# sgl-project/rbg

Measured on AMD Instinct MI355X. Metric: output tok/s (llama-3-8b P/D-disagg serving, KV migration over xGMI), higher is better.
Workload: dtype bf16; 1 GPU; model=llama-3-8b, global_batch=128, seq_len=2048, parallelism=pd1 (1 prefill + 1 decode, prefill colocated with decode0)

## Files before the change

rbg_amd/models/llama.py:

```python
from __future__ import annotations

import math
from dataclasses import dataclass
from typing import Optional

import torch
import torch.nn as nn

from .. import ops
from ..engine.config import ModelConfig
from ..engine.kv_cache import PagedKVCache


@dataclass
class ForwardBatch:
    mode: str
    positions: torch.Tensor
    slot_mapping: torch.Tensor
    cu_seqlens: Optional[torch.Tensor] = None
    cu_seqlens_k: Optional[torch.Tensor] = None
    kv_gather_slots: Optional[torch.Tensor] = None
    block_tables: Optional[torch.Tensor] = None
    context_lens: Optional[torch.Tensor] = None
    decode_num_splits: int = 0
# ... 67 lines not shown

    def recv_prev(self, shape, dtype, device) -> torch.Tensor:
        from ..parallel.comm import from_wire, wire_dtype
        t = torch.empty(shape, dtype=wire_dtype(dtype, device),
                        device=device)
        torch.distributed.recv(t, src=self._lane_rank(self.stage - 1))
        return from_wire(t, dtype)

    def broadcast_tokens(self, t: torch.Tensor) -> torch.Tensor:
        src = self.ranks[(self.size - 1) * self.tp_size]
        torch.distributed.broadcast(t, src=src, group=self.group)
        return t


class LlamaAttention(nn.Module):
    def __init__(self, cfg: ModelConfig, layer_idx: int, tp: TPContext,
                 device, dtype, gen):
        super().__init__()
        self.cfg = cfg
        self.layer_idx = layer_idx
        self.tp = tp
        assert cfg.num_heads % tp.size == 0 and cfg.num_kv_heads % tp.size == 0, \
            "TP degree must divide head counts"
        self.heads = cfg.num_heads // tp.size
        self.kv_heads = cfg.num_kv_heads // tp.size
        self.head_dim = cfg.head_dim
        self.scale = 1.0 / math.sqrt(cfg.head_dim)
        q_out = self.heads * cfg.head_dim
        kv_out = self.kv_heads * cfg.head_dim
        full_q = cfg.num_heads * cfg.head_dim
        full_kv = cfg.num_kv_heads * cfg.head_dim
        wq = _linear_weight(full_q, cfg.hidden_size, device, dtype, gen,
                            shard_dim=0, tp_size=tp.size, tp_rank=tp.rank)
        wk = _linear_weight(full_kv, cfg.hidden_size, device, dtype, gen,
                            shard_dim=0, tp_size=tp.size, tp_rank=tp.rank)
        wv = _linear_weight(full_kv, cfg.hidden_size, device, dtype, gen,
                            shard_dim=0, tp_size=tp.size, tp_rank=tp.rank)
        self.wqkv = nn.Parameter(torch.cat([wq, wk, wv], dim=0),
                                 requires_grad=False)
        self.wo = _linear_weight(cfg.hidden_size, full_q, device, dtype, gen,
                                 shard_dim=1, tp_size=tp.size,
                                 tp_rank=tp.rank)
        self.q_out, self.kv_out = q_out, kv_out
        self.q_norm = self.k_norm = None
        if cfg.qk_norm:
            self.q_norm = nn.Parameter(torch.ones(cfg.head_dim, device=device,
                                                  dtype=dtype),
                                       requires_grad=False)
            self.k_norm = nn.Parameter(torch.ones(cfg.head_dim, device=device,
                                                  dtype=dtype),
                                       requires_grad=False)

    def forward(self, x: torch.Tensor, batch: ForwardBatch,
                kv: PagedKVCache, cos_sin: torch.Tensor) -> torch.Tensor:
        T = x.shape[0]
        qkv = ops.linear(x, self.wqkv)
        q = qkv[:, :self.q_out]
        k = qkv[:, self.q_out:self.q_out + self.kv_out]
        v = qkv[:, self.q_out + self.kv_out:]
        if self.q_norm is not None:
            q = ops.rmsnorm(q.contiguous().view(-1, self.head_dim),
                            self.q_norm,
                            self.cfg.rms_eps).view(T, self.q_out)
            k = ops.rmsnorm(k.contiguous().view(-1, self.head_dim),
                            self.k_norm,
                            self.cfg.rms_eps).view(T, self.kv_out)
            v = v.clone(memory_format=torch.contiguous_format)
        key_cache = kv.key_cache(self.layer_idx)
        value_cache = kv.value_cache(self.layer_idx)
        fp8 = kv.fp8
        if fp8:
            ops.rope_store_kv(q, k, v, key_cache, value_cache, cos_sin,
                              batch.positions, batch.slot_mapping,
                              kv.k_scale_log2, kv.v_scale_log2)
        else:
            ops.rope_store_kv(q, k, v, key_cache, value_cache, cos_sin,
                              batch.positions, batch.slot_mapping)
        q3 = q.view(T, self.heads, self.head_dim)
        if batch.mode == "prefill":
            if fp8:
                if batch.kv_gather_slots is None:
                    raise RuntimeError("an fp8 KV pool prefills through the "
                                       "gather path: kv_gather_slots unset")
                k_full = ops.kv_gather_dequant(
                    key_cache, batch.kv_gather_slots, kv.k_scale_log2)
                v_full = ops.kv_gather_dequant(
                    value_cache, batch.kv_gather_slots, kv.v_scale_log2)
                o = ops.prefill_attention(q3, k_full, v_full,
                                          batch.cu_seqlens, self.scale,
                                          batch.cu_seqlens_k)
            elif batch.kv_gather_slots is not None:
                ps = key_cache.shape[2]
                slots = batch.kv_gather_slots.long()
                pages, offs = slots // ps, slots % ps
                k_full = key_cache[pages, :, offs]
                v_full = value_cache[pages, :, offs]
                o = ops.prefill_attention(q3, k_full, v_full,
                                          batch.cu_seqlens, self.scale,
                                          batch.cu_seqlens_k)
            else:
                o = ops.prefill_attention(
                    q3, k.view(T, self.kv_heads, self.head_dim),
                    v.view(T, self.kv_heads, self.head_dim),
                    batch.cu_seqlens, self.scale)
        elif fp8:
            o = ops.decode_attention(q3, key_cache, value_cache,
                                     batch.block_tables, batch.context_lens,
                                     self.scale,
                                     num_splits=batch.decode_num_splits,
                                     k_scale_log2=kv.k_scale_log2,
                                     v_scale_log2=kv.v_scale_log2)
        else:
            o = ops.decode_attention(q3, key_cache, value_cache,
                                     batch.block_tables, batch.context_lens,
                                     self.scale,
                                     num_splits=batch.decode_num_splits)
        out = ops.linear(o.view(T, self.q_out).contiguous(), self.wo)
        return self.tp.all_reduce(out)


class LlamaMLP(nn.Module):
    def __init__(self, cfg: ModelConfig, tp: TPContext, device, dtype, gen):
        super().__init__()
        self.tp = tp
        assert cfg.intermediate_size % tp.size == 0
        inter = cfg.intermediate_size // tp.size
        wg = _linear_weight(cfg.intermediate_size, cfg.hidden_size, device,
                            dtype, gen, shard_dim=0, tp_size=tp.size,
                            tp_rank=tp.rank)
        wu = _linear_weight(cfg.intermediate_size, cfg.hidden_size, device,
                            dtype, gen, shard_dim=0, tp_size=tp.size,
                            tp_rank=tp.rank)
        self.w_gate_up = nn.Parameter(torch.cat([wg, wu], dim=0),
                                      requires_grad=False)
        self.w_down = _linear_weight(cfg.hidden_size, cfg.intermediate_size,
                                     device, dtype, gen, shard_dim=1,
                                     tp_size=tp.size, tp_rank=tp.rank)
        self.inter = inter

    def forward(self, x: torch.Tensor) -> torch.Tensor:
        gu = ops.linear(x, self.w_gate_up)
        h = ops.silu_mul(gu)
        return self.tp.all_reduce(ops.linear(h, self.w_down))


class LlamaLayer(nn.Module):
    def __init__(self, cfg: ModelConfig, layer_idx: int, tp: TPContext,
                 device, dtype, gen):
        super().__init__()
        self.attn = LlamaAttention(cfg, layer_idx, tp, device, dtype, gen)
        self.mlp = LlamaMLP(cfg, tp, device, dtype, gen)
        self.input_norm = nn.Parameter(
            torch.ones(cfg.hidden_size, device=device, dtype=dtype),
            requires_grad=False)
        self.post_norm = nn.Parameter(
            torch.ones(cfg.hidden_size, device=device, dtype=dtype),
            requires_grad=False)
        self.eps = cfg.rms_eps

    def forward(self, x: torch.Tensor, residual: Optional[torch.Tensor],
                batch: ForwardBatch, kv: PagedKVCache,
                cos_sin: torch.Tensor):
        if residual is None:
            residual = x.clone()
            h = ops.rmsnorm(x, self.input_norm, self.eps)
        else:
            ops.fused_add_rmsnorm(x, residual, self.input_norm, self.eps)
            h = x
        h = self.attn(h, batch, kv, cos_sin)
        ops.fused_add_rmsnorm(h, residual, self.post_norm, self.eps)
        h = self.mlp(h)
        return h, residual


class LlamaForCausalLM(nn.Module):
    def __init__(self, cfg: ModelConfig, device: torch.device,
                 tp: Optional[TPContext] = None, base_seed: int = 1234,
                 pp: Optional[PPContext] = None):
        super().__init__()
        self.cfg = cfg
        self.tp = tp or TPContext()
        self.pp = pp or PPContext()
        self.base_seed = base_seed
        self.device = device
        dtype = torch.bfloat16
        self.dtype = dtype

        def _gen(tag: int) -> torch.Generator:
            g = torch.Generator(device=device)
            g.manual_seed(base_seed * 1000003 + tag)
            return g

        L = cfg.num_layers
        assert L % self.pp.size == 0, "PP degree must divide layer count"
        per = L // self.pp.size
        self.layer_start = self.pp.stage * per
        self.layer_end = self.layer_start + per
        self.embed = None
        if self.pp.first:
            self.embed = nn.Parameter(
                torch.empty(cfg.vocab_size, cfg.hidden_size, device=device,
                            dtype=dtype).normal_(0, 0.02, generator=_gen(0)),
                requires_grad=False)
        self.layers = nn.ModuleList([
            LlamaLayer(cfg, i - self.layer_start, self.tp, device, dtype,
                       _gen(1 + i))
            for i in range(self.layer_start, self.layer_end)])
        self.final_norm = None
        self.lm_head = None
        if self.pp.last:
            self.final_norm = nn.Parameter(
                torch.ones(cfg.hidden_size, device=device, dtype=dtype),
                requires_grad=False)
            self.lm_head = _linear_weight(cfg.vocab_size, cfg.hidden_size,
                                          device, dtype, _gen(L + 1))
        self.cos_sin = ops.build_cos_sin_table(
            cfg.head_dim, cfg.max_position, cfg.rope_theta,
            device=device)

    @property
    def num_local_layers(self) -> int:
        return self.layer_end - self.layer_start

    @torch.inference_mode()
    def forward(self, tokens: torch.Tensor, batch: ForwardBatch,
                kv: PagedKVCache,
                hidden: Optional[torch.Tensor] = None) -> torch.Tensor:
        if self.pp.first:
            x = self.embed[tokens.long()]
        else:
            assert hidden is not None, "non-first PP stage needs hidden"
            x = hidden
        residual = None
        for layer in self.layers:
            x, residual = layer(x, residual, batch, kv, self.cos_sin)
        x = x + residual
        if not self.pp.last:
            return x
        x = ops.rmsnorm(x, self.final_norm, self.cfg.rms_eps)
        return x

    @torch.inference_mode()
    def logits(self, hidden: torch.Tensor,
               gather_idx: Optional[torch.Tensor] = None) -> torch.Tensor:
        if gather_idx is not None:
            hidden = hidden[gather_idx.long()]
        return torch.nn.functional.linear(hidden, self.lm_head).float()

    def reload_weights(self, seed: int) -> None:
        fresh = LlamaForCausalLM(self.cfg, self.device, self.tp,
                                 base_seed=seed, pp=self.pp)
        with torch.no_grad():
            for p, q in zip(self.parameters(), fresh.parameters()):
                p.copy_(q)
        del fresh
        if self.device.type == "cuda":
            torch.cuda.empty_cache()
        if self.tp.size > 1:
            torch.distributed.barrier(group=self.tp.group)
```

rbg_amd/ops/__init__.py:

```python
from __future__ import annotations

import os

import torch

from . import reference

_hip = None
_hip_err: Exception | None = None
try:
    from . import _hip_ops as _hip
except Exception as e:
    _hip_err = e

HAVE_HIP = _hip is not None


def _check_stale() -> None:
    import hashlib
    here = os.path.dirname(os.path.abspath(__file__))
    stamp = os.path.join(here, "_hip_ops.srchash")
    if not os.path.exists(stamp):
        return
    h = hashlib.sha256()
    hip_dir = os.path.join(here, "hip")
    for name in sorted(os.listdir(hip_dir)):
        if name.endswith("_hip.hip"):
            continue
        if name.endswith((".hip", ".cpp", ".h")):
            with open(os.path.join(hip_dir, name), "rb") as f:
                h.update(name.encode() + b"\0" + f.read() + b"\0")
    with open(stamp) as f:
        recorded = f.read().strip()
    if recorded and recorded != h.hexdigest():
        raise RuntimeError(
            "rbg_amd HIP extension is STALE: kernel sources changed after "
            "the last build.  Rebuild in-tree: PYTORCH_ROCM_ARCH=gfx950 "
            "python setup.py build_ext --inplace")


if HAVE_HIP and torch.cuda.is_available():
    _check_stale()


def _require_hip():
    if _hip is None:
        raise RuntimeError(
            "rbg_amd HIP extension is not built but a GPU tensor was passed. "
            "Build it in-tree: PYTORCH_ROCM_ARCH=gfx950 python setup.py "
            f"build_ext --inplace (import error: {_hip_err!r})")
    return _hip


def _on_gpu(t: torch.Tensor) -> bool:
    return t.is_cuda


SKINNY_GEMM = int(os.environ.get("RBG_SKINNY_GEMM", "1"))


def linear(x: torch.Tensor, w: torch.Tensor) -> torch.Tensor:
    if (SKINNY_GEMM and _on_gpu(x) and x.dim() == 2 and
            x.dtype == torch.bfloat16 and 1 <= x.shape[0] <= 128 and
            w.shape[0] % 32 == 0 and x.shape[1] % 512 == 0 and
            (w.shape[0] <= 4608 or
             (x.shape[0] <= 64 and w.shape[0] <= 8192))):
        return _require_hip().skinny_gemm(
            x if x.is_contiguous() else x.contiguous(), w)
    return torch.nn.functional.linear(x, w)


def rmsnorm(x: torch.Tensor, weight: torch.Tensor, eps: float) -> torch.Tensor:
    if _on_gpu(x):
        return _require_hip().rmsnorm(x, weight, eps)
    return reference.rmsnorm(x, weight, eps)


def fused_add_rmsnorm(x: torch.Tensor, residual: torch.Tensor,
                      weight: torch.Tensor, eps: float) -> None:
    if _on_gpu(x):
        _require_hip().fused_add_rmsnorm(x, residual, weight, eps)
        return
    reference.fused_add_rmsnorm(x, residual, weight, eps)


def silu_mul(x: torch.Tensor) -> torch.Tensor:
    if _on_gpu(x):
        return _require_hip().silu_mul(x)
    return reference.silu_mul(x)


FP8 = torch.float8_e4m3fn
KV_CACHE_DTYPES = reference.KV_CACHE_DTYPES
KV_SCALE_LOG2_RANGE = reference.KV_SCALE_LOG2_RANGE
check_kv_scale_log2 = reference.check_kv_scale_log2


def _is_fp8_pair(key_cache, value_cache) -> bool:
    if key_cache.dtype != value_cache.dtype:
        raise ValueError("key_cache is %s but value_cache is %s" % (
            key_cache.dtype, value_cache.dtype))
    return key_cache.dtype == FP8


def rope_store_kv(q, k, v, key_cache, value_cache, cos_sin, positions,
                  slot_mapping, k_scale_log2: int = 0,
                  v_scale_log2: int = 0) -> None:
    if _is_fp8_pair(key_cache, value_cache):
        check_kv_scale_log2(k_scale_log2, "kv_k_scale_log2")
        check_kv_scale_log2(v_scale_log2, "kv_v_scale_log2")
        if _on_gpu(q):
            _require_hip().rope_store_kv_fp8(
                q, k, v, key_cache, value_cache, cos_sin, positions,
                slot_mapping, k_scale_log2, v_scale_log2)
            return
        reference.rope_store_kv(q, k, v, key_cache, value_cache, cos_sin,
                                positions, slot_mapping, k_scale_log2,
                                v_scale_log2)
        return
    if _on_gpu(q):
        _require_hip().rope_store_kv(q, k, v, key_cache, value_cache,
                                     cos_sin, positions, slot_mapping)
# ... 102 lines not shown
```

rbg_amd/ops/hip/bindings.cpp:

```cpp
#include <torch/extension.h>
#include <ATen/hip/HIPContext.h>

#include <hip/hip_runtime.h>

#include <algorithm>
#include <cmath>
#include <cstring>
#include <vector>

extern "C" {
void launch_rmsnorm(void*, void*, const void*, float, int, int, hipStream_t);
void launch_fused_add_rmsnorm(void*, void*, const void*, float, int, int,
                              hipStream_t);
void launch_silu_mul(void*, const void*, int, int, hipStream_t);
void launch_rope_store_kv(void*, void*, const void*, void*, void*,
                          const void*, const void*, const void*, int, int,
                          int, int, int, int, int, hipStream_t);
void launch_decode_attention(void*, void*, void*, const void*, const void*,
                             const void*, const void*, const void*, float,
                             int, int, int, int, int, int, int, int,
                             hipStream_t);
void launch_prefill_attention(void*, const void*, const void*, const void*,
                              const void*, const void*, float, int, int, int,
                              int, int, int, hipStream_t);
void launch_mfma_probe(void*, const void*, const void*, int, int, hipStream_t);
void launch_mfma_probe32(void*, const void*, const void*, int, int, int,
                         hipStream_t);
void launch_skinny_gemm(void*, void*, const void*, const void*, int, int,
                        int, int, hipStream_t);
void launch_reduce_splits(void*, const void*, int, long, hipStream_t);
void launch_kv_peer_copy(void*, const void*, const void*, const void*, int,
                         int, int, long, long, long, long, hipStream_t);
void launch_xgmi_allreduce(void*, const void*, void**, void**, int, int,
                           long, hipStream_t);
void launch_sample(void*, void*, const void*, const void*, const void*,
                   const void*, const void*, const void*, const void*, int,
                   int, hipStream_t);
void launch_rope_store_kv_fp8(void*, void*, const void*, void*, void*,
                              const void*, const void*, const void*, int, int,
                              int, int, int, int, float, float, hipStream_t);
void launch_kv_gather_dequant(void*, const void*, const void*, long, int, int,
                              int, float, hipStream_t);
void launch_decode_attention_fp8(void*, void*, void*, const void*, const void*,
                                 const void*, const void*, const void*, float,
                                 float, int, int, int, int, int, int,
                                 hipStream_t);
long xgmi_allreduce_signal_bytes();
long xgmi_allreduce_error_offset();
long xgmi_allreduce_counter_offset();
}

namespace {

hipStream_t current_stream() {
  return at::hip::getCurrentHIPStream().stream();
}

void check_bf16_contig(const torch::Tensor& t, const char* name) {
  TORCH_CHECK(t.is_cuda(), name, " must be on GPU");
  TORCH_CHECK(t.scalar_type() == torch::kBFloat16, name, " must be bf16");
  TORCH_CHECK(t.is_contiguous(), name, " must be contiguous");
}

void check_i32_gpu(const torch::Tensor& t, const char* name) {
  TORCH_CHECK(t.is_cuda(), name, " must be on GPU");
  TORCH_CHECK(t.scalar_type() == torch::kInt32, name, " must be int32");
  TORCH_CHECK(t.is_contiguous(), name, " must be contiguous");
}

void check_kv_caches(const torch::Tensor& key_cache,
                     const torch::Tensor& value_cache) {
  check_bf16_contig(key_cache, "key_cache");
  check_bf16_contig(value_cache, "value_cache");
  TORCH_CHECK(key_cache.dim() == 4,
              "key_cache must be [pages, KVH, page_size, head_dim]");
  TORCH_CHECK(value_cache.sizes() == key_cache.sizes(),
              "key_cache/value_cache shape mismatch");
  const int64_t page_size = key_cache.size(2);
  TORCH_CHECK(page_size > 0 && (page_size & (page_size - 1)) == 0,
              "page_size must be a power of two");
  TORCH_CHECK(key_cache.size(1) > 0, "cache needs at least one KV head");
  TORCH_CHECK(key_cache.size(3) > 0 && key_cache.size(3) % 8 == 0,
              "cache head_dim must be a multiple of 8");
// ... 317 lines not shown
  rowsliced3(q, "q");
  rowsliced3(k, "k");
  rowsliced3(v, "v");
  TORCH_CHECK(k.stride(0) == v.stride(0), "k/v stride mismatch");
  TORCH_CHECK(q.size(2) == 128, "head_dim must be 128");
  TORCH_CHECK(block_info.scalar_type() == torch::kInt32, "block_info int32");
  TORCH_CHECK(seq_lens.scalar_type() == torch::kInt32, "seq_lens int32");
  const int nblocks = block_info.size(0);
  const int num_q_heads = q.size(1);
  const int num_kv_heads = k.size(1);
  auto out = torch::empty({q.size(0), (int64_t)num_q_heads, (int64_t)128},
                          q.options());
  launch_prefill_attention(out.data_ptr(), q.data_ptr(), k.data_ptr(),
                           v.data_ptr(), block_info.data_ptr(),
                           seq_lens.data_ptr(), (float)scale, nblocks,
                           num_q_heads, num_kv_heads, (int)swz,
                           (int)q.stride(0), (int)k.stride(0),
                           current_stream());
  return out;
}

torch::Tensor mfma_probe(torch::Tensor a, torch::Tensor b, int64_t a_split,
                         int64_t b_split) {
  auto d = torch::zeros({16, 16}, a.options().dtype(torch::kFloat32));
  launch_mfma_probe(d.data_ptr(), a.data_ptr(), b.data_ptr(), (int)a_split,
                    (int)b_split, current_stream());
  return d;
}

torch::Tensor mfma_probe32(torch::Tensor a, torch::Tensor b, int64_t a_split,
                           int64_t b_split, int64_t dmap) {
  auto d = torch::zeros({32, 32}, a.options().dtype(torch::kFloat32));
  launch_mfma_probe32(d.data_ptr(), a.data_ptr(), b.data_ptr(), (int)a_split,
                      (int)b_split, (int)dmap, current_stream());
  return d;
}

}

static int pick_gemm_splits(int N, int K) {
  const int n_groups = N >> 5;
  for (int s : {8, 4, 2})
    if (n_groups * s <= 512 && n_groups * s >= 192 && K % (s * 256) == 0)
      return s;
  for (int s : {4, 2})
    if (n_groups * s >= 128 && K % (s * 256) == 0) return s;
  return 1;
}

bool skinny_gemm_supported(int64_t M, int64_t N, int64_t K) {
  return M >= 1 && M <= 256 && (N % 32) == 0 && (K % 256) == 0;
}

torch::Tensor skinny_gemm(torch::Tensor a, torch::Tensor w,
                          int64_t force_splits = 0) {
  check_bf16_contig(a, "a");
  check_bf16_contig(w, "w");
  TORCH_CHECK(a.dim() == 2 && w.dim() == 2, "a and w must be 2-D");
  TORCH_CHECK(a.device() == w.device(), "a/w device mismatch");
  const int64_t M = a.size(0), K = a.size(1), N = w.size(0);
  TORCH_CHECK(w.size(1) == K, "K mismatch");
  TORCH_CHECK(skinny_gemm_supported(M, N, K), "unsupported skinny shape");
  TORCH_CHECK(force_splits == 0 || force_splits == 1 || force_splits == 2 ||
                  force_splits == 4 || force_splits == 8,
              "force_splits must be 0 (auto), 1, 2, 4 or 8");
  TORCH_CHECK(force_splits == 0 || K % (force_splits * 256) == 0,
              "K must be a multiple of force_splits * 256");
  auto c = torch::empty({M, N}, a.options());
  const int splits = force_splits > 0 ? (int)force_splits
                                      : pick_gemm_splits((int)N, (int)K);
  torch::Tensor ws;
  void* wsp = nullptr;
  if (splits > 1) {
    ws = torch::empty({splits, M, N}, a.options().dtype(torch::kFloat32));
    wsp = ws.data_ptr();
  }
  launch_skinny_gemm(c.data_ptr(), wsp, a.data_ptr(), w.data_ptr(), (int)M,
                     (int)N, (int)K, splits, current_stream());
  if (splits > 1)
    launch_reduce_splits(c.data_ptr(), wsp, splits, (long)(M * N),
                         current_stream());
  return c;
}

std::vector<torch::Tensor> sample(torch::Tensor logits,
                                  torch::Tensor temperature,
                                  torch::Tensor top_k, torch::Tensor top_p,
                                  torch::Tensor min_p, torch::Tensor seed,
                                  torch::Tensor pos) {
  TORCH_CHECK(logits.is_cuda(), "logits must be on GPU");
  TORCH_CHECK(logits.scalar_type() == torch::kFloat32, "logits must be fp32");
  TORCH_CHECK(logits.dim() == 2, "logits must be [n, V]");
  TORCH_CHECK(logits.is_contiguous(), "logits must be contiguous");
  const int64_t n = logits.size(0), V = logits.size(1);
  TORCH_CHECK(V >= 1, "V must be >= 1");
  TORCH_CHECK(V <= INT32_MAX && n <= INT32_MAX, "n and V must fit int32");
  auto check_param = [&](const torch::Tensor& t, torch::ScalarType dt,
                         const char* name) {
    TORCH_CHECK(t.is_cuda() && t.device() == logits.device(), name,
                " must be on the logits' device");
    TORCH_CHECK(t.scalar_type() == dt, name, " has the wrong dtype");
    TORCH_CHECK(t.dim() == 1 && t.size(0) == n, name,
                " must have one entry per row");
    TORCH_CHECK(t.is_contiguous(), name, " must be contiguous");
  };
  check_param(temperature, torch::kFloat32, "temperature");
  check_param(top_k, torch::kInt32, "top_k");
  check_param(top_p, torch::kFloat32, "top_p");
  check_param(min_p, torch::kFloat32, "min_p");
  check_param(seed, torch::kInt64, "seed");
  check_param(pos, torch::kInt32, "pos");
  auto tokens = torch::empty({n}, logits.options().dtype(torch::kInt64));
  auto kept = torch::empty({n}, logits.options().dtype(torch::kInt32));
  if (n == 0) return {tokens, kept};
  launch_sample(tokens.data_ptr(), kept.data_ptr(), logits.data_ptr(),
                temperature.data_ptr(), top_k.data_ptr(), top_p.data_ptr(),
                min_p.data_ptr(), seed.data_ptr(), pos.data_ptr(), (int)n,
                (int)V, current_stream());
  return {tokens, kept};
}


torch::Tensor ipc_alloc_bf16(std::vector<int64_t> sizes) {
  int64_t numel = 1;
  for (auto s : sizes) numel *= s;
  void* ptr = nullptr;
  hipError_t err = hipMalloc(&ptr, numel * 2);
  TORCH_CHECK(err == hipSuccess, "hipMalloc(", numel * 2,
              " B) failed: ", hipGetErrorString(err));
  int dev = 0;
  (void)hipGetDevice(&dev);
  auto opts = torch::TensorOptions()
                  .dtype(torch::kBFloat16)
                  .device(torch::kCUDA, dev);
  return torch::from_blob(
      ptr, sizes, [](void* p) { (void)hipFree(p); }, opts);
// ... 99 lines not shown
  unsigned err_word = 0;
  char* base = reinterpret_cast<char*>(sig_ptr);
  (void)hipMemcpy(&err_word, base + xgmi_allreduce_error_offset(),
                  sizeof(unsigned), hipMemcpyDeviceToHost);
  return err_word;
}

torch::Tensor ar_dump_signals(int64_t sig_ptr) {
  long n = xgmi_allreduce_signal_bytes() / 4;
  auto t = torch::empty({n}, torch::TensorOptions().dtype(torch::kInt32));
  (void)hipMemcpy(t.data_ptr(), reinterpret_cast<void*>(sig_ptr), n * 4,
                  hipMemcpyDeviceToHost);
  return t;
}

torch::Tensor xgmi_allreduce(torch::Tensor inp,
                             std::vector<int64_t> sig_ptrs,
                             std::vector<int64_t> data_ptrs, int64_t rank) {
  check_bf16_contig(inp, "inp");
  const int world = (int)sig_ptrs.size();
  TORCH_CHECK(world >= 1 && world <= 8 &&
                  data_ptrs.size() == (size_t)world && rank >= 0 &&
                  rank < world,
              "bad world/rank");
  TORCH_CHECK(inp.numel() % 8 == 0, "numel must be a multiple of 8");
  auto out = torch::empty_like(inp);
  void* sp[8];
  void* dp[8];
  for (int i = 0; i < world; ++i) {
    sp[i] = reinterpret_cast<void*>(sig_ptrs[i]);
    dp[i] = reinterpret_cast<void*>(data_ptrs[i]);
  }
  launch_xgmi_allreduce(out.data_ptr(), inp.data_ptr(), sp, dp, world,
                        (int)rank, (long)inp.numel(), current_stream());
  return out;
}

PYBIND11_MODULE(TORCH_EXTENSION_NAME, m) {
  m.def("rmsnorm", &rmsnorm, "RMSNorm (bf16)");
  m.def("fused_add_rmsnorm", &fused_add_rmsnorm, "x,residual += ; rmsnorm");
  m.def("silu_mul", &silu_mul, "silu(gate)*up");
  m.def("rope_store_kv", &rope_store_kv, "RoPE + paged KV write");
  m.def("decode_attention", &decode_attention, "paged flash-decode");
  m.def("rope_store_kv_fp8", &rope_store_kv_fp8,
        "RoPE + quantising (e4m3) paged KV write");
  m.def("kv_gather_dequant", &kv_gather_dequant,
        "gather e4m3 cache rows by slot -> bf16 [Tkv, KVH, D]");
  m.def("decode_attention_fp8", &decode_attention_fp8,
        "paged flash-decode over an e4m3 cache (page-pair MFMA)");
  m.def("prefill_attention", &prefill_attention, "varlen causal flash prefill");
  m.def("mfma_probe", &mfma_probe, "MFMA layout probe");
  m.def("mfma_probe32", &mfma_probe32, "32x32x16 MFMA layout probe");
  m.def("skinny_gemm", &skinny_gemm, "decode-shape GEMM (M<=128)",
        py::arg("a"), py::arg("w"), py::arg("force_splits") = 0);
  m.def("sample", &sample,
        "seeded top-k/min-p/top-p Gumbel-max sampler -> (tokens, num_kept)");
  m.def("ipc_alloc_bf16", &ipc_alloc_bf16,
        "hipMalloc-backed bf16 tensor (IPC-exportable base allocation)",
        py::call_guard<py::gil_scoped_release>());
  m.def("ipc_alloc", &ipc_alloc,
        "hipMalloc-backed tensor of any dtype (IPC-exportable allocation)",
        py::call_guard<py::gil_scoped_release>());
  m.def("kv_ipc_export", &kv_ipc_export, "hipIpcGetMemHandle of a KV pool");
  m.def("kv_ipc_open", &kv_ipc_open,
        "map a peer KV pool (lazy xGMI peer access)",
        py::call_guard<py::gil_scoped_release>());
  m.def("kv_ipc_close", &kv_ipc_close, "unmap a peer KV pool",
        py::call_guard<py::gil_scoped_release>());
  m.def("kv_peer_copy", &kv_peer_copy,
        "gather local pages -> scatter into peer pool over xGMI",
        py::call_guard<py::gil_scoped_release>());
  m.def("ar_alloc_signals", &ar_alloc_signals,
        "uncached signal buffer for the xGMI all-reduce");
  m.def("ar_export_ptr", &ar_export_ptr, "hipIpc handle of a raw pointer");
  m.def("ar_error_flag", &ar_error_flag, "read the all-reduce error word");
  m.def("ar_dump_signals", &ar_dump_signals, "debug: dump the signal block");
  m.def("ar_counter_offset", &xgmi_allreduce_counter_offset);
  m.def("xgmi_allreduce", &xgmi_allreduce,
        "one-shot all-reduce over peer-mapped HBM (graph-capturable)");
}
```

rbg_amd/ops/hip/rmsnorm.hip:

```cpp
#include "common.h"

namespace {

template <bool FUSED_ADD>
__global__ void rmsnorm_kernel(__hip_bfloat16* __restrict__ out,
                               __hip_bfloat16* __restrict__ input,
                               __hip_bfloat16* __restrict__ residual,
                               const __hip_bfloat16* __restrict__ w,
                               const float eps, const int hidden) {
  const int row = blockIdx.x;
  const int tid = threadIdx.x;
  const int nthreads = blockDim.x;
  __shared__ float red[8];
  __shared__ float s_inv;

  __hip_bfloat16* in_row = input + (size_t)row * hidden;
  __hip_bfloat16* res_row =
      FUSED_ADD ? residual + (size_t)row * hidden : nullptr;
  __hip_bfloat16* out_row = out + (size_t)row * hidden;

  const int nvec = hidden / 8;
  float ss = 0.f;
  for (int i = tid; i < nvec; i += nthreads) {
    Bf16x8U xv;
    xv.u = *reinterpret_cast<const uint4*>(in_row + i * 8);
    if (FUSED_ADD) {
      Bf16x8U rv;
      rv.u = *reinterpret_cast<const uint4*>(res_row + i * 8);
#pragma unroll
      for (int j = 0; j < 8; ++j) {
        float s = bf2f(xv.e[j]) + bf2f(rv.e[j]);
        xv.e[j] = f2bf(s);
        ss += s * s;
      }
      *reinterpret_cast<uint4*>(res_row + i * 8) = xv.u;
    } else {
#pragma unroll
      for (int j = 0; j < 8; ++j) {
        float s = bf2f(xv.e[j]);
        ss += s * s;
      }
    }
  }
  const int lane = tid & 63, wave = tid >> 6;
  ss = wave_sum(ss);
  if (lane == 0) red[wave] = ss;
  __syncthreads();
  if (tid == 0) {
    float total = 0.f;
    for (int wv = 0; wv < (nthreads >> 6); ++wv) total += red[wv];
    s_inv = rsqrtf(total / hidden + eps);
  }
  __syncthreads();
  const float inv = s_inv;

  const __hip_bfloat16* src = FUSED_ADD ? res_row : in_row;
  for (int i = tid; i < nvec; i += nthreads) {
    Bf16x8U xv, wv, ov;
    xv.u = *reinterpret_cast<const uint4*>(src + i * 8);
    wv.u = *reinterpret_cast<const uint4*>(w + i * 8);
#pragma unroll
    for (int j = 0; j < 8; ++j)
      ov.e[j] = f2bf(bf2f(xv.e[j]) * inv * bf2f(wv.e[j]));
    *reinterpret_cast<uint4*>(out_row + i * 8) = ov.u;
  }
}

}

extern "C" {

void launch_rmsnorm(void* out, void* input, const void* weight, float eps,
                    int tokens, int hidden, hipStream_t stream) {
  dim3 grid(tokens), block(256);
  hipLaunchKernelGGL(rmsnorm_kernel<false>, grid, block, 0, stream,
                     (__hip_bfloat16*)out, (__hip_bfloat16*)input,
                     (__hip_bfloat16*)nullptr, (const __hip_bfloat16*)weight,
                     eps, hidden);
}

void launch_fused_add_rmsnorm(void* input, void* residual, const void* weight,
                              float eps, int tokens, int hidden,
                              hipStream_t stream) {
  dim3 grid(tokens), block(256);
  hipLaunchKernelGGL(rmsnorm_kernel<true>, grid, block, 0, stream,
                     (__hip_bfloat16*)input, (__hip_bfloat16*)input,
                     (__hip_bfloat16*)residual, (const __hip_bfloat16*)weight,
                     eps, hidden);
}

}
```

rbg_amd/ops/hip/skinny_gemm.hip:

```cpp
#include "common.h"

typedef __attribute__((ext_vector_type(8))) __bf16 gg_bf8;

DEV_INLINE gg_bf8 lds_frag(const __hip_bfloat16* p) {
  union { uint4 u; gg_bf8 v; } cvt;
  cvt.u = *reinterpret_cast<const uint4*>(p);
  return cvt.v;
}

#define SG_KSTEP 64
#define SG_LDS_PITCH (SG_KSTEP + 8)
#define SG_NT 256

template <int M_TILES, int SPLITS>
__global__ __launch_bounds__(SG_NT, 3) void skinny_gemm_kernel(
    const __hip_bfloat16* __restrict__ a,
    const __hip_bfloat16* __restrict__ w,
    __hip_bfloat16* __restrict__ c,
    float* __restrict__ ws,
    const int M, const int N, const int K) {
  const int n_groups = N >> 5;
  const int n_group = blockIdx.x % n_groups;
  const int split = blockIdx.x / n_groups;
  const int tid = threadIdx.x;
// ... 96 lines not shown
  __hip_bfloat16* buf1 = lds.stage[1];

  SG_ISSUE(0, wreg0, a00, a01, a02, a03, a04, a05, a06, a07);
  SG_ISSUE(1, wreg1, a10, a11, a12, a13, a14, a15, a16, a17);
  SG_WRITE(buf0, wreg0, a00, a01, a02, a03, a04, a05, a06, a07);
  SG_ISSUE(2, wreg0, a00, a01, a02, a03, a04, a05, a06, a07);

  for (int step = 0; step < nsteps; step += 2) {
    __syncthreads();
    compute(buf0);
    SG_WRITE(buf1, wreg1, a10, a11, a12, a13, a14, a15, a16, a17);
    SG_ISSUE(step + 3, wreg1, a10, a11, a12, a13, a14, a15, a16, a17);
    __syncthreads();
    compute(buf1);
    SG_WRITE(buf0, wreg0, a00, a01, a02, a03, a04, a05, a06, a07);
    SG_ISSUE(step + 4, wreg0, a00, a01, a02, a03, a04, a05, a06, a07);
  }
#undef SG_ISSUE
#undef SG_WRITE
#undef SG_ABASE
#undef SG_LD
#undef SG_AST

  __syncthreads();
#pragma unroll
  for (int mt = 0; mt < M_TILES; ++mt) {
    F32x4U u;
    u.v = acc[mt];
#pragma unroll
    for (int r = 0; r < 4; ++r)
      lds.red[wave][mt * 256 + r * 64 + lane] = u.e[r];
  }
  __syncthreads();

  const int elems = M_TILES * 256 * 2;
  for (int e = tid; e < elems; e += SG_NT) {
    const int nt = e >= M_TILES * 256;
    const int ee = e - nt * M_TILES * 256;
    const float v = lds.red[nt][ee] + lds.red[2 + nt][ee];
    const int l64 = ee & 63;
    const int reg = (ee >> 6) & 3;
    const int mt = ee >> 8;
    const int m = mt * 16 + ((l64 >> 4) << 2) + reg;
    if (m < M) {
      const int n = (n_group << 5) + (nt << 4) + (l64 & 15);
      if (SPLITS == 1)
        c[(size_t)m * N + n] = f2bf(v);
      else
        ws[((size_t)split * M + m) * N + n] = v;
    }
  }
}

__global__ void reduce_splits_kernel(const float* __restrict__ ws,
                                     __hip_bfloat16* __restrict__ c,
                                     const int splits, const long mn) {
  const long i = (long)blockIdx.x * blockDim.x + threadIdx.x;
  if (i >= mn) return;
  float v = 0.f;
  for (int s = 0; s < splits; ++s) v += ws[(size_t)s * mn + i];
  c[i] = f2bf(v);
}


extern "C" void launch_skinny_gemm(void* c, void* ws, const void* a,
                                   const void* w, int M, int N, int K,
                                   int splits, hipStream_t stream) {
  const dim3 grid((N >> 5) * splits), block(SG_NT);
  const __hip_bfloat16* ap = (const __hip_bfloat16*)a;
  const __hip_bfloat16* wp = (const __hip_bfloat16*)w;
  __hip_bfloat16* cp = (__hip_bfloat16*)c;
  float* wsp = (float*)ws;
  const int m_tiles = (M + 15) >> 4;

#define LAUNCH_MT(MT)                                                        \
  do {                                                                       \
    if (splits == 1)                                                         \
      skinny_gemm_kernel<MT, 1><<<grid, block, 0, stream>>>(                 \
          ap, wp, cp, nullptr, M, N, K);                                     \
    else if (splits == 2)                                                    \
      skinny_gemm_kernel<MT, 2><<<grid, block, 0, stream>>>(                 \
          ap, wp, cp, wsp, M, N, K);                                         \
    else if (splits == 4)                                                    \
      skinny_gemm_kernel<MT, 4><<<grid, block, 0, stream>>>(                 \
          ap, wp, cp, wsp, M, N, K);                                         \
    else                                                                     \
      skinny_gemm_kernel<MT, 8><<<grid, block, 0, stream>>>(                 \
          ap, wp, cp, wsp, M, N, K);                                         \
  } while (0)

  if (m_tiles <= 1) LAUNCH_MT(1);
  else if (m_tiles <= 2) LAUNCH_MT(2);
  else if (m_tiles <= 4) LAUNCH_MT(4);
  else if (m_tiles <= 8) LAUNCH_MT(8);
  else LAUNCH_MT(16);
#undef LAUNCH_MT
}

extern "C" void launch_reduce_splits(void* c, const void* ws, int splits,
                                     long mn, hipStream_t stream) {
  const int threads = 256;
  reduce_splits_kernel<<<dim3((mn + threads - 1) / threads), dim3(threads),
                         0, stream>>>((const float*)ws, (__hip_bfloat16*)c,
                                      splits, mn);
}
```

Baseline: 10380 tok/s.

## Fuse split-K reduction into add-RMSNorm and add wide-panel skinny GEMM

Folds the split-K partial-sum reduction into the following fused add+RMSNorm kernel, and moves each layer's next input norm into the MLP down-projection epilogue, so one reduce kernel and one norm launch per linear are removed. It also adds a 64-column, 512-thread skinny GEMM variant with double-buffered LDS staging, chosen automatically for M>32. The goal is fewer decode kernel launches and less memory traffic, at the cost of a new untested kernel path and more complex layer wiring when TP size is 1.

```diff
diff --git a/rbg_amd/models/llama.py b/rbg_amd/models/llama.py
--- a/rbg_amd/models/llama.py
+++ b/rbg_amd/models/llama.py
@@ -143,7 +143,8 @@
                                        requires_grad=False)
 
     def forward(self, x: torch.Tensor, batch: ForwardBatch,
-                kv: PagedKVCache, cos_sin: torch.Tensor) -> torch.Tensor:
+                kv: PagedKVCache, cos_sin: torch.Tensor,
+                add_norm=None) -> torch.Tensor:
         T = x.shape[0]
         qkv = ops.linear(x, self.wqkv)
         q = qkv[:, :self.q_out]
@@ -206,8 +207,10 @@
                                      batch.block_tables, batch.context_lens,
                                      self.scale,
                                      num_splits=batch.decode_num_splits)
-        out = ops.linear(o.view(T, self.q_out).contiguous(), self.wo)
-        return self.tp.all_reduce(out)
+        o = o.view(T, self.q_out).contiguous()
+        if add_norm is not None:
+            return ops.linear_add_rmsnorm(o, self.wo, *add_norm)
+        return self.tp.all_reduce(ops.linear(o, self.wo))
 
 
 class LlamaMLP(nn.Module):
@@ -229,9 +232,11 @@
                                      tp_size=tp.size, tp_rank=tp.rank)
         self.inter = inter
 
-    def forward(self, x: torch.Tensor) -> torch.Tensor:
+    def forward(self, x: torch.Tensor, add_norm=None) -> torch.Tensor:
         gu = ops.linear(x, self.w_gate_up)
         h = ops.silu_mul(gu)
+        if add_norm is not None:
+            return ops.linear_add_rmsnorm(h, self.w_down, *add_norm)
         return self.tp.all_reduce(ops.linear(h, self.w_down))
 
 
@@ -248,6 +253,9 @@
             torch.ones(cfg.hidden_size, device=device, dtype=dtype),
             requires_grad=False)
         self.eps = cfg.rms_eps
+        self.fuse_norms = False
+        self.next_input_norm: tuple = ()
+        self.input_prenormed = False
 
     def forward(self, x: torch.Tensor, residual: Optional[torch.Tensor],
                 batch: ForwardBatch, kv: PagedKVCache,
@@ -255,13 +263,21 @@
         if residual is None:
             residual = x.clone()
             h = ops.rmsnorm(x, self.input_norm, self.eps)
+        elif self.input_prenormed:
+            h = x
         else:
             ops.fused_add_rmsnorm(x, residual, self.input_norm, self.eps)
             h = x
-        h = self.attn(h, batch, kv, cos_sin)
-        ops.fused_add_rmsnorm(h, residual, self.post_norm, self.eps)
-        h = self.mlp(h)
-        return h, residual
+        if not self.fuse_norms:
+            h = self.attn(h, batch, kv, cos_sin)
+            ops.fused_add_rmsnorm(h, residual, self.post_norm, self.eps)
+            return self.mlp(h), residual
+        h = self.attn(h, batch, kv, cos_sin,
+                      add_norm=(residual, self.post_norm, self.eps))
+        if self.next_input_norm:
+            return self.mlp(h, add_norm=(residual, self.next_input_norm[0],
+                                         self.eps)), residual
+        return self.mlp(h), residual
 
 
 class LlamaForCausalLM(nn.Module):
@@ -297,6 +313,7 @@
             LlamaLayer(cfg, i - self.layer_start, self.tp, device, dtype,
                        _gen(1 + i))
             for i in range(self.layer_start, self.layer_end)])
+        self.link_norm_fusion(self.tp.size == 1)
         self.final_norm = None
         self.lm_head = None
         if self.pp.last:
@@ -308,6 +325,14 @@
         self.cos_sin = ops.build_cos_sin_table(
             cfg.head_dim, cfg.max_position, cfg.rope_theta,
             device=device)
+
+    def link_norm_fusion(self, on: bool) -> None:
+        layers = list(self.layers)
+        for i, layer in enumerate(layers):
+            nxt = layers[i + 1] if on and i + 1 < len(layers) else None
+            layer.fuse_norms = on
+            layer.input_prenormed = on and i > 0
+            layer.next_input_norm = () if nxt is None else (nxt.input_norm,)
 
     @property
     def num_local_layers(self) -> int:
diff --git a/rbg_amd/ops/__init__.py b/rbg_amd/ops/__init__.py
--- a/rbg_amd/ops/__init__.py
+++ b/rbg_amd/ops/__init__.py
@@ -60,14 +60,30 @@
 
 
 def linear(x: torch.Tensor, w: torch.Tensor) -> torch.Tensor:
-    if (SKINNY_GEMM and _on_gpu(x) and x.dim() == 2 and
-            x.dtype == torch.bfloat16 and 1 <= x.shape[0] <= 128 and
-            w.shape[0] % 32 == 0 and x.shape[1] % 512 == 0 and
-            (w.shape[0] <= 4608 or
-             (x.shape[0] <= 64 and w.shape[0] <= 8192))):
+    if _use_skinny_gemm(x, w):
         return _require_hip().skinny_gemm(
             x if x.is_contiguous() else x.contiguous(), w)
     return torch.nn.functional.linear(x, w)
+
+
+def _use_skinny_gemm(x: torch.Tensor, w: torch.Tensor) -> bool:
+    return bool(SKINNY_GEMM and _on_gpu(x) and x.dim() == 2 and
+                x.dtype == torch.bfloat16 and 1 <= x.shape[0] <= 128 and
+                w.shape[0] % 32 == 0 and x.shape[1] % 512 == 0 and
+                (w.shape[0] <= 4608 or
+                 (x.shape[0] <= 64 and w.shape[0] <= 8192)))
+
+
+def linear_add_rmsnorm(x: torch.Tensor, w: torch.Tensor,
+                       residual: torch.Tensor, norm_weight: torch.Tensor,
+                       eps: float) -> torch.Tensor:
+    if _use_skinny_gemm(x, w):
+        return _require_hip().skinny_gemm_add_rmsnorm(
+            x if x.is_contiguous() else x.contiguous(), w, residual,
+            norm_weight, eps)
+    h = linear(x, w)
+    fused_add_rmsnorm(h, residual, norm_weight, eps)
+    return h
 
 
 def rmsnorm(x: torch.Tensor, weight: torch.Tensor, eps: float) -> torch.Tensor:
diff --git a/rbg_amd/ops/hip/bindings.cpp b/rbg_amd/ops/hip/bindings.cpp
--- a/rbg_amd/ops/hip/bindings.cpp
+++ b/rbg_amd/ops/hip/bindings.cpp
@@ -28,7 +28,11 @@
                          hipStream_t);
 void launch_skinny_gemm(void*, void*, const void*, const void*, int, int,
                         int, int, hipStream_t);
+void launch_skinny_gemm_wide(void*, void*, const void*, const void*, int, int,
+                             int, int, hipStream_t);
 void launch_reduce_splits(void*, const void*, int, long, hipStream_t);
+void launch_fold_add_rmsnorm(void*, const void*, void*, const void*, float,
+                             int, int, int, hipStream_t);
 void launch_kv_peer_copy(void*, const void*, const void*, const void*, int,
                          int, int, long, long, long, long, hipStream_t);
 void launch_xgmi_allreduce(void*, const void*, void**, void**, int, int,
@@ -452,8 +456,19 @@
   return M >= 1 && M <= 256 && (N % 32) == 0 && (K % 256) == 0;
 }
 
-torch::Tensor skinny_gemm(torch::Tensor a, torch::Tensor w,
-                          int64_t force_splits = 0) {
+bool skinny_gemm_wide_supported(int64_t M, int64_t N) {
+  return M >= 1 && M <= 128 && (N % 64) == 0;
+}
+
+static int pick_gemm_panel(int64_t M, int64_t N) {
+  return M > 32 && skinny_gemm_wide_supported(M, N) ? 64 : 32;
+}
+
+namespace {
+
+int skinny_gemm_launch(const torch::Tensor& a, const torch::Tensor& w,
+                       int64_t force_splits, int64_t panel, torch::Tensor& c,
+                       torch::Tensor& ws) {
   check_bf16_contig(a, "a");
   check_bf16_contig(w, "w");
   TORCH_CHECK(a.dim() == 2 && w.dim() == 2, "a and w must be 2-D");
@@ -466,22 +481,74 @@
               "force_splits must be 0 (auto), 1, 2, 4 or 8");
   TORCH_CHECK(force_splits == 0 || K % (force_splits * 256) == 0,
               "K must be a multiple of force_splits * 256");
-  auto c = torch::empty({M, N}, a.options());
+  TORCH_CHECK(panel == 0 || panel == 32 || panel == 64,
+              "panel must be 0 (auto), 32 or 64");
+  TORCH_CHECK(panel != 64 || skinny_gemm_wide_supported(M, N),
+              "panel 64 needs M <= 128 and N % 64 == 0");
   const int splits = force_splits > 0 ? (int)force_splits
                                       : pick_gemm_splits((int)N, (int)K);
-  torch::Tensor ws;
+  if (panel == 0) panel = pick_gemm_panel(M, N);
+  void* cp = nullptr;
   void* wsp = nullptr;
   if (splits > 1) {
     ws = torch::empty({splits, M, N}, a.options().dtype(torch::kFloat32));
     wsp = ws.data_ptr();
+  } else {
+    c = torch::empty({M, N}, a.options());
+    cp = c.data_ptr();
   }
-  launch_skinny_gemm(c.data_ptr(), wsp, a.data_ptr(), w.data_ptr(), (int)M,
-                     (int)N, (int)K, splits, current_stream());
-  if (splits > 1)
-    launch_reduce_splits(c.data_ptr(), wsp, splits, (long)(M * N),
-                         current_stream());
+  (panel == 64 ? launch_skinny_gemm_wide : launch_skinny_gemm)(
+      cp, wsp, a.data_ptr(), w.data_ptr(), (int)M, (int)N, (int)K, splits,
+      current_stream());
+  return splits;
+}
+
+}
+
+torch::Tensor skinny_gemm(torch::Tensor a, torch::Tensor w,
+                          int64_t force_splits = 0, int64_t panel = 0) {
+  torch::Tensor c, ws;
+  const int splits = skinny_gemm_launch(a, w, force_splits, panel, c, ws);
+  if (splits > 1) {
+    c = torch::empty({a.size(0), w.size(0)}, a.options());
+    launch_reduce_splits(c.data_ptr(), ws.data_ptr(), splits,
+                         (long)c.numel(), current_stream());
+  }
   return c;
 }
+
+torch::Tensor skinny_gemm_add_rmsnorm(torch::Tensor a, torch::Tensor w,
+                                      torch::Tensor residual,
+                                      torch::Tensor norm_weight, double eps,
+                                      int64_t force_splits = 0,
+                                      int64_t panel = 0) {
+  check_bf16_contig(residual, "residual");
+  check_bf16_contig(norm_weight, "norm_weight");
+  TORCH_CHECK(a.dim() == 2 && w.dim() == 2, "a and w must be 2-D");
+  TORCH_CHECK(residual.dim() == 2 && residual.size(0) == a.size(0) &&
+                  residual.size(1) == w.size(0),
+              "residual must be [M, N]");
+  TORCH_CHECK(norm_weight.numel() == w.size(0),
+              "norm_weight must have N elements");
+  TORCH_CHECK(residual.device() == a.device() &&
+                  norm_weight.device() == a.device(),
+              "a/residual/norm_weight device mismatch");
+  torch::Tensor c, ws;
+  const int splits = skinny_gemm_launch(a, w, force_splits, panel, c, ws);
+  const int M = (int)a.size(0), N = (int)w.size(0);
+  if (splits == 1) {
+    launch_fused_add_rmsnorm(c.data_ptr(), residual.data_ptr(),
+                             norm_weight.data_ptr(), (float)eps, M, N,
+                             current_stream());
+    return c;
+  }
+  c = torch::empty({a.size(0), w.size(0)}, a.options());
+  launch_fold_add_rmsnorm(c.data_ptr(), ws.data_ptr(), residual.data_ptr(),
+                          norm_weight.data_ptr(), (float)eps, splits, M, N,
+                          current_stream());
+  return c;
+}
+
 
 std::vector<torch::Tensor> sample(torch::Tensor logits,
                                   torch::Tensor temperature,
@@ -687,7 +754,14 @@
   m.def("mfma_probe", &mfma_probe, "MFMA layout probe");
   m.def("mfma_probe32", &mfma_probe32, "32x32x16 MFMA layout probe");
   m.def("skinny_gemm", &skinny_gemm, "decode-shape GEMM (M<=128)",
-        py::arg("a"), py::arg("w"), py::arg("force_splits") = 0);
+        py::arg("a"), py::arg("w"), py::arg("force_splits") = 0,
+        py::arg("panel") = 0);
+  m.def("skinny_gemm_add_rmsnorm", &skinny_gemm_add_rmsnorm,
+        "skinny_gemm + fused_add_rmsnorm with the split-K fold inside the "
+        "norm kernel; returns h, updates residual in place",
+        py::arg("a"), py::arg("w"), py::arg("residual"),
+        py::arg("norm_weight"), py::arg("eps"), py::arg("force_splits") = 0,
+        py::arg("panel") = 0);
   m.def("sample", &sample,
         "seeded top-k/min-p/top-p Gumbel-max sampler -> (tokens, num_kept)");
   m.def("ipc_alloc_bf16", &ipc_alloc_bf16,
diff --git a/rbg_amd/ops/hip/rmsnorm.hip b/rbg_amd/ops/hip/rmsnorm.hip
--- a/rbg_amd/ops/hip/rmsnorm.hip
+++ b/rbg_amd/ops/hip/rmsnorm.hip
@@ -2,19 +2,24 @@
 
 namespace {
 
-template <bool FUSED_ADD>
+enum { NORM_PLAIN = 0, NORM_FUSED_ADD = 1, NORM_FOLD_ADD = 2 };
+
+template <int MODE, int SPLITS = 1>
 __global__ void rmsnorm_kernel(__hip_bfloat16* __restrict__ out,
                                __hip_bfloat16* __restrict__ input,
                                __hip_bfloat16* __restrict__ residual,
                                const __hip_bfloat16* __restrict__ w,
+                               const float* __restrict__ ws,
                                const float eps, const int hidden) {
+  constexpr bool FUSED_ADD = MODE != NORM_PLAIN;
   const int row = blockIdx.x;
   const int tid = threadIdx.x;
   const int nthreads = blockDim.x;
   __shared__ float red[8];
   __shared__ float s_inv;
 
-  __hip_bfloat16* in_row = input + (size_t)row * hidden;
+  __hip_bfloat16* in_row =
+      MODE == NORM_FOLD_ADD ? nullptr : input + (size_t)row * hidden;
   __hip_bfloat16* res_row =
       FUSED_ADD ? residual + (size_t)row * hidden : nullptr;
   __hip_bfloat16* out_row = out + (size_t)row * hidden;
@@ -23,7 +28,26 @@
   float ss = 0.f;
   for (int i = tid; i < nvec; i += nthreads) {
     Bf16x8U xv;
-    xv.u = *reinterpret_cast<const uint4*>(in_row + i * 8);
+    if (MODE == NORM_FOLD_ADD) {
+      const size_t mn = (size_t)gridDim.x * hidden;
+      const float* p = ws + (size_t)row * hidden + i * 8;
+      float4 lo[SPLITS], hi[SPLITS];
+#pragma unroll
+      for (int s = 0; s < SPLITS; ++s) {
+        lo[s] = *reinterpret_cast<const float4*>(p + s * mn);
+        hi[s] = *reinterpret_cast<const float4*>(p + s * mn + 4);
+      }
+      float v[8] = {0.f, 0.f, 0.f, 0.f, 0.f, 0.f, 0.f, 0.f};
+#pragma unroll
+      for (int s = 0; s < SPLITS; ++s) {
+        v[0] += lo[s].x; v[1] += lo[s].y; v[2] += lo[s].z; v[3] += lo[s].w;
+        v[4] += hi[s].x; v[5] += hi[s].y; v[6] += hi[s].z; v[7] += hi[s].w;
+      }
+#pragma unroll
+      for (int j = 0; j < 8; ++j) xv.e[j] = f2bf(v[j]);
+    } else {
+      xv.u = *reinterpret_cast<const uint4*>(in_row + i * 8);
+    }
     if (FUSED_ADD) {
       Bf16x8U rv;
       rv.u = *reinterpret_cast<const uint4*>(res_row + i * 8);
@@ -73,20 +97,36 @@
 void launch_rmsnorm(void* out, void* input, const void* weight, float eps,
                     int tokens, int hidden, hipStream_t stream) {
   dim3 grid(tokens), block(256);
-  hipLaunchKernelGGL(rmsnorm_kernel<false>, grid, block, 0, stream,
+  hipLaunchKernelGGL(rmsnorm_kernel<NORM_PLAIN>, grid, block, 0, stream,
                      (__hip_bfloat16*)out, (__hip_bfloat16*)input,
                      (__hip_bfloat16*)nullptr, (const __hip_bfloat16*)weight,
-                     eps, hidden);
+                     (const float*)nullptr, eps, hidden);
 }
 
 void launch_fused_add_rmsnorm(void* input, void* residual, const void* weight,
                               float eps, int tokens, int hidden,
                               hipStream_t stream) {
   dim3 grid(tokens), block(256);
-  hipLaunchKernelGGL(rmsnorm_kernel<true>, grid, block, 0, stream,
+  hipLaunchKernelGGL(rmsnorm_kernel<NORM_FUSED_ADD>, grid, block, 0, stream,
                      (__hip_bfloat16*)input, (__hip_bfloat16*)input,
                      (__hip_bfloat16*)residual, (const __hip_bfloat16*)weight,
-                     eps, hidden);
+                     (const float*)nullptr, eps, hidden);
+}
+
+void launch_fold_add_rmsnorm(void* out, const void* ws, void* residual,
+                             const void* weight, float eps, int splits,
+                             int tokens, int hidden, hipStream_t stream) {
+  dim3 grid(tokens), block(256);
+#define LAUNCH_FOLD(S)                                                       \
+  hipLaunchKernelGGL((rmsnorm_kernel<NORM_FOLD_ADD, S>), grid, block, 0,      \
+                     stream, (__hip_bfloat16*)out, (__hip_bfloat16*)nullptr, \
+                     (__hip_bfloat16*)residual,                              \
+                     (const __hip_bfloat16*)weight, (const float*)ws, eps,   \
+                     hidden)
+  if (splits == 2) LAUNCH_FOLD(2);
+  else if (splits == 4) LAUNCH_FOLD(4);
+  else LAUNCH_FOLD(8);
+#undef LAUNCH_FOLD
 }
 
 }
diff --git a/rbg_amd/ops/hip/skinny_gemm.hip b/rbg_amd/ops/hip/skinny_gemm.hip
--- a/rbg_amd/ops/hip/skinny_gemm.hip
+++ b/rbg_amd/ops/hip/skinny_gemm.hip
@@ -172,6 +172,163 @@
   }
 }
 
+#define SGW_NT 512
+
+template <int MTW, int SPLITS>
+__global__ __launch_bounds__(SGW_NT) void skinny_gemm_wide_kernel(
+    const __hip_bfloat16* __restrict__ a,
+    const __hip_bfloat16* __restrict__ w,
+    __hip_bfloat16* __restrict__ c,
+    float* __restrict__ ws,
+    const int M, const int N, const int K) {
+  const int n_groups = N >> 6;
+  const int n_group = blockIdx.x % n_groups;
+  const int split = blockIdx.x / n_groups;
+  const int tid = threadIdx.x;
+  const int wave = tid >> 6;
+  const int lane = tid & 63;
+  const int gl = lane & 15;
+  const int gslice = lane >> 4;
+
+  const int row_group = wave & 3;
+  const int k_slice = wave >> 2;
+  const int k_wg = K / SPLITS;
+  const int k0 = split * k_wg;
+  const int nsteps = k_wg / SG_KSTEP;
+
+  constexpr int A_ROWS = MTW * 64;
+  constexpr int BUF = (64 + A_ROWS) * SG_LDS_PITCH;
+  __shared__ union {
+    __hip_bfloat16 stage[2][BUF];
+    float red[4][MTW * 4 * 256];
+  } lds;
+
+  const int srow = tid >> 3, schk = (tid & 7) * 8;
+  const __hip_bfloat16* wbase =
+      w + (size_t)((n_group << 6) + srow) * K + schk;
+  const __hip_bfloat16* ab0 = a + (size_t)min(srow, M - 1) * K + schk;
+  const __hip_bfloat16* ab1 = a + (size_t)min(srow + 64, M - 1) * K + schk;
+
+  uint4 w0, w1, w2, w3;
+  uint4 a00, a01 = {}, a10, a11 = {};
+
+#define SGW_KB(step) (k0 + min(step, nsteps - 1) * SG_KSTEP)
+#define SGW_LD(p, kb) (*reinterpret_cast<const uint4*>((p) + (kb)))
+#define SGW_ISSUE_A(step, x0, x1)                                           \
+  do {                                                                      \
+    const int kb = SGW_KB(step);                                            \
+    x0 = SGW_LD(ab0, kb);                                                   \
+    if (MTW > 1) x1 = SGW_LD(ab1, kb);                                      \
+  } while (0)
+#define SGW_ISSUE_W(step, wr) wr = SGW_LD(wbase, SGW_KB(step))
+#define SGW_WRITE(st, wr, x0, x1)                                           \
+  do {                                                                      \
+    *reinterpret_cast<uint4*>(&st[srow * SG_LDS_PITCH + schk]) = wr;        \
+    *reinterpret_cast<uint4*>(&st[(64 + srow) * SG_LDS_PITCH + schk]) = x0; \
+    if (MTW > 1)                                                            \
+      *reinterpret_cast<uint4*>(&st[(128 + srow) * SG_LDS_PITCH + schk]) =  \
+          x1;                                                               \
+  } while (0)
+
+  f32x4 acc[MTW][4];
+#pragma unroll
+  for (int mt = 0; mt < MTW; ++mt)
+#pragma unroll
+    for (int nt = 0; nt < 4; ++nt) acc[mt][nt] = {0.f, 0.f, 0.f, 0.f};
+
+  const int kf = k_slice * 32 + gslice * 8;
+  auto compute = [&](const __hip_bfloat16* st) {
+    const gg_bf8 wf0 = lds_frag(&st[gl * SG_LDS_PITCH + kf]);
+    const gg_bf8 wf1 = lds_frag(&st[(16 + gl) * SG_LDS_PITCH + kf]);
+    const gg_bf8 wf2 = lds_frag(&st[(32 + gl) * SG_LDS_PITCH + kf]);
+    const gg_bf8 wf3 = lds_frag(&st[(48 + gl) * SG_LDS_PITCH + kf]);
+#pragma unroll
+    for (int mt = 0; mt < MTW; ++mt) {
+      const gg_bf8 af = lds_frag(
+          &st[(64 + (row_group * MTW + mt) * 16 + gl) * SG_LDS_PITCH + kf]);
+      acc[mt][0] = __builtin_amdgcn_mfma_f32_16x16x32_bf16(af, wf0,
+                                                           acc[mt][0], 0, 0, 0);
+      acc[mt][1] = __builtin_amdgcn_mfma_f32_16x16x32_bf16(af, wf1,
+                                                           acc[mt][1], 0, 0, 0);
+      acc[mt][2] = __builtin_amdgcn_mfma_f32_16x16x32_bf16(af, wf2,
+                                                           acc[mt][2], 0, 0, 0);
+      acc[mt][3] = __builtin_amdgcn_mfma_f32_16x16x32_bf16(af, wf3,
+                                                           acc[mt][3], 0, 0, 0);
+    }
+  };
+
+  __hip_bfloat16* buf0 = lds.stage[0];
+  __hip_bfloat16* buf1 = lds.stage[1];
+
+  SGW_ISSUE_A(0, a00, a01);
+  SGW_ISSUE_W(0, w0);
+  SGW_ISSUE_A(1, a10, a11);
+  SGW_ISSUE_W(1, w1);
+  SGW_ISSUE_W(2, w2);
+  SGW_ISSUE_W(3, w3);
+  SGW_WRITE(buf0, w0, a00, a01);
+  SGW_ISSUE_A(2, a00, a01);
+  SGW_ISSUE_W(4, w0);
+
+#define SGW_STEP(t, cur, nxt, wr, x0, x1)                                   \
+  do {                                                                      \
+    __syncthreads();                                                        \
+    compute(cur);                                                           \
+    SGW_WRITE(nxt, wr, x0, x1);                                             \
+    SGW_ISSUE_A((t) + 3, x0, x1);                                           \
+    SGW_ISSUE_W((t) + 5, wr);                                               \
+  } while (0)
+  for (int step = 0; step < nsteps; step += 4) {
+    SGW_STEP(step, buf0, buf1, w1, a10, a11);
+    SGW_STEP(step + 1, buf1, buf0, w2, a00, a01);
+    SGW_STEP(step + 2, buf0, buf1, w3, a10, a11);
+    SGW_STEP(step + 3, buf1, buf0, w0, a00, a01);
+  }
+#undef SGW_STEP
+#undef SGW_WRITE
+#undef SGW_ISSUE_W
+#undef SGW_ISSUE_A
+#undef SGW_LD
+#undef SGW_KB
+
+  __syncthreads();
+  if (k_slice == 1) {
+#pragma unroll
+    for (int mt = 0; mt < MTW; ++mt)
+#pragma unroll
+      for (int nt = 0; nt < 4; ++nt) {
+        F32x4U u;
+        u.v = acc[mt][nt];
+#pragma unroll
+        for (int r = 0; r < 4; ++r)
+          lds.red[row_group][(mt * 4 + nt) * 256 + r * 64 + lane] = u.e[r];
+      }
+  }
+  __syncthreads();
+  if (k_slice == 0) {
+#pragma unroll
+    for (int mt = 0; mt < MTW; ++mt)
+#pragma unroll
+      for (int nt = 0; nt < 4; ++nt) {
+        F32x4U u;
+        u.v = acc[mt][nt];
+        const int n = (n_group << 6) + (nt << 4) + gl;
+#pragma unroll
+        for (int r = 0; r < 4; ++r) {
+          const float v =
+              u.e[r] + lds.red[row_group][(mt * 4 + nt) * 256 + r * 64 + lane];
+          const int m = (row_group * MTW + mt) * 16 + (gslice << 2) + r;
+          if (m < M) {
+            if (SPLITS == 1)
+              c[(size_t)m * N + n] = f2bf(v);
+            else
+              ws[((size_t)split * M + m) * N + n] = v;
+          }
+        }
+      }
+  }
+}
+
 __global__ void reduce_splits_kernel(const float* __restrict__ ws,
                                      __hip_bfloat16* __restrict__ c,
                                      const int splits, const long mn) {
@@ -217,6 +374,36 @@
 #undef LAUNCH_MT
 }
 
+extern "C" void launch_skinny_gemm_wide(void* c, void* ws, const void* a,
+                                        const void* w, int M, int N, int K,
+                                        int splits, hipStream_t stream) {
+  const dim3 grid((N >> 6) * splits), block(SGW_NT);
+  const __hip_bfloat16* ap = (const __hip_bfloat16*)a;
+  const __hip_bfloat16* wp = (const __hip_bfloat16*)w;
+  __hip_bfloat16* cp = (__hip_bfloat16*)c;
+  float* wsp = (float*)ws;
+
+#define LAUNCH_MTW(MTW)                                                      \
+  do {                                                                       \
+    if (splits == 1)                                                         \
+      skinny_gemm_wide_kernel<MTW, 1><<<grid, block, 0, stream>>>(           \
+          ap, wp, cp, nullptr, M, N, K);                                     \
+    else if (splits == 2)                                                    \
+      skinny_gemm_wide_kernel<MTW, 2><<<grid, block, 0, stream>>>(           \
+          ap, wp, cp, wsp, M, N, K);                                         \
+    else if (splits == 4)                                                    \
+      skinny_gemm_wide_kernel<MTW, 4><<<grid, block, 0, stream>>>(           \
+          ap, wp, cp, wsp, M, N, K);                                         \
+    else                                                                     \
+      skinny_gemm_wide_kernel<MTW, 8><<<grid, block, 0, stream>>>(           \
+          ap, wp, cp, wsp, M, N, K);                                         \
+  } while (0)
+
+  if (M <= 64) LAUNCH_MTW(1);
+  else LAUNCH_MTW(2);
+#undef LAUNCH_MTW
+}
+
 extern "C" void launch_reduce_splits(void* c, const void* ws, int splits,
                                      long mn, hipStream_t stream) {
   const int threads = 256;
```

Result: faster. 10940 tok/s (median of 6 runs) (+5.4%).
